# CSMaus/DefectDetection_viaObjectDetection

Hardware: AMD Instinct MI355X
Metric: images/sec @640x640 b32 YOLOv8s-seg (higher is better)
Workload: dtype fp16; 1 GPU; YOLOv8s-seg inference (forward + NMS + masks), 32 synthetic 640x640 B-scans per GPU per step, nc=1, seeded synthetic weights; pipelined throughput, 2 batch(es) in flight (ms_per_step is the step period, not a latency); inputs rotate over 8 HBM-resident batches (300 MiB); input_batches=8, per_gpu_batch=32, global_batch=32, parallelism=batch-sharded x1, no collective, max_det=300, engines_in_flight=2, stream_lanes_per_engine=1

## Files before the change

defectdetection_viaobjectdetection_amd/_capi.py:

```python
from __future__ import annotations

import ctypes as C
import os

_HERE = os.path.dirname(os.path.abspath(__file__))
LIB_PATH = os.path.join(_HERE, "lib", "libmi355yolo.so")


class M355Error(RuntimeError):
    """Raised when a libmi355yolo call returns a negative status."""


class ModelDesc(C.Structure):
    _fields_ = [("scale", C.c_int), ("nc", C.c_int), ("in_h", C.c_int), ("in_w", C.c_int),
                ("max_batch", C.c_int)]


class ConvInfo(C.Structure):
    _fields_ = [("name", C.c_char * 64), ("cin", C.c_int), ("cout", C.c_int), ("k", C.c_int),
                ("stride", C.c_int), ("has_bn", C.c_int), ("transposed", C.c_int), ("act", C.c_int),
                ("groups", C.c_int)]


class OpInfo(C.Structure):
# ... 95 lines not shown
    "m355_get_raw_head": (C.c_int, [_P, C.POINTER(_P), C.POINTER(C.c_int)]),
    "m355_copy_raw_head": (C.c_int, [_P, C.c_int, _P, _P]),
    "m355_set_keep_raw": (C.c_int, [_P, C.c_int]),
    "m355_postprocess": (C.c_int, [_P, _P, _P, C.c_int, C.c_float, C.c_float, C.c_int, _P, _P, _P, _P]),
    "m355_conv2d_fwd": (C.c_int, [_P, C.c_int, C.c_int, C.c_int, C.c_int, _P, _P, C.c_int, C.c_int, C.c_int,
                                  C.c_int, _P, _P, C.c_int, C.c_int, _P]),
    "m355_c2f_c32_fwd": (C.c_int, [_P, C.c_int, C.c_int, C.c_int, _P, _P, _P, _P, _P, _P, C.c_int, _P, _P]),
    "m355_bneck_pair_fwd": (C.c_int, [_P, C.c_int, C.c_int, C.c_int, C.c_int, C.c_int, _P, _P, _P, _P, C.c_int, _P, C.c_int, _P]),
    "m355_conv3x3_blockdiag_fwd": (C.c_int, [_P, C.c_int, C.c_int, C.c_int, C.c_int, C.c_int, _P, _P, _P, _P, _P, C.c_int, C.c_int, _P]),
    "m355_planes_diag_pack": (C.c_long, [C.c_int, _P, _P, _P, _P, C.c_long]),
    "m355_s2c64_cv1_fwd": (C.c_int, [_P, C.c_int, C.c_int, C.c_int, _P, _P, _P, _P, _P, _P]),
    "m355_stem_s2c32_cv1_fwd": (C.c_int, [_P, C.c_int, C.c_int, C.c_int, _P, _P, _P, _P, _P, _P, _P, C.c_int, _P]),
    "m355_proto_phase_fwd": (C.c_int, [_P, C.c_int, C.c_int, C.c_int, _P, _P, _P, _P, _P, _P, _P, _P]),
    "m355_head_tail_fwd": (C.c_int, [_P, C.c_int, C.c_int, C.c_int, C.c_int, C.c_float, _P, _P, _P, _P, _P, _P, _P, C.c_int, C.c_int, _P]),
    "m355_tal_assign_launch": (C.c_int, [_P, _P, _P, _P, _P, _P, C.c_int32, C.c_int32, C.c_int32, C.c_int32, _P, _P, _P, _P, _P, _P]),
    "m355_conv2d_dgrad": (C.c_int, [_P, C.c_int, C.c_int, C.c_int, C.c_int, _P, C.c_int, C.c_int, C.c_int, _P, _P]),
    "m355_conv2d_wgrad": (C.c_int, [_P, _P, C.c_int, C.c_int, C.c_int, C.c_int, C.c_int, C.c_int, C.c_int, _P, _P]),
    "m355_bn_silu_train_fwd": (C.c_int, [_P, C.c_int, C.c_int, C.c_int, C.c_int, _P, _P, C.c_float, C.c_int, _P, _P, _P, _P, _P]),
    "m355_bn_silu_train_bwd": (C.c_int, [_P, _P, C.c_int, C.c_int, C.c_int, C.c_int, _P, _P, _P, _P, C.c_int, _P, _P, _P, _P]),
    "m355_bn_workspace_floats": (C.c_size_t, [C.c_int]),
    "m355_wgrad_workspace_bytes": (C.c_size_t, [C.c_int32, C.c_int32, C.c_int32, C.c_int32, C.c_int32, C.c_int32]),
    "m355_grad_sumsq_workspace_floats": (C.c_size_t, []),
    "m355_convt2x2_fwd": (C.c_int, [_P, C.c_int, C.c_int, C.c_int, C.c_int, _P, _P, C.c_int, _P, _P]),
    "m355_stem_fwd": (C.c_int, [_P, C.c_int, C.c_int, C.c_int, _P, _P, C.c_int, _P, _P]),
    "m355_stem6_fwd": (C.c_int, [_P, C.c_int, C.c_int, C.c_int, _P, _P, C.c_int, _P, _P]),
    "m355_dwconv3x3_fwd": (C.c_int, [_P, C.c_int, C.c_int, C.c_int, C.c_int, C.c_int, _P, _P, C.c_int, _P, C.c_int, _P]),
    "m355_psa_attn_fwd": (C.c_int, [_P, C.c_int, C.c_int, C.c_int, C.c_int, C.c_int, C.c_int, _P, _P, _P, _P]),
    "m355_sppf_pool": (C.c_int, [_P, C.c_int, C.c_int, C.c_int, C.c_int, _P, _P]),
    "m355_upsample2x": (C.c_int, [_P, C.c_int, C.c_int, C.c_int, C.c_int, _P, _P]),
    "m355_head_decode": (C.c_int, [_P, C.c_int, C.c_int, C.c_int, C.c_int, _P, _P]),
    "m355_head_decode_ex": (C.c_int, [_P, C.c_int, C.c_int, C.c_int, C.c_int, C.c_int, _P, _P]),
    "m355_nms": (C.c_int, [_P, C.c_int, C.c_int, C.c_int, C.c_int, C.c_float, C.c_float, C.c_int, _P, _P, _P]),
    "m355_conv_launch": (C.c_int, [C.POINTER(ConvLaunchArgs), _P]),
    "m355_wgrad_launch": (C.c_int, [C.POINTER(WgradLaunchArgs), _P]),
    "m355_bn_train_fwd_launch": (C.c_int, [_P, C.c_int64, C.c_int32, C.c_int32, _P, _P, C.c_float, C.c_int32, _P, C.c_int32,
                                           _P, C.c_int32, _P, _P, _P, _P, _P, C.c_float, _P]),
    "m355_bn_train_bwd_launch": (C.c_int, [_P, _P, C.c_int64, C.c_int32, C.c_int32, C.c_int32, _P, _P, _P, _P, C.c_int32,
                                           _P, C.c_int32, _P, _P, _P]),
    "m355_adamw_step": (C.c_int, [_P, _P, _P, _P, _P, _P, C.c_int64, C.c_float, C.c_float, C.c_float, C.c_float, C.c_float,
                                  C.c_float, C.c_int32, C.c_float, C.c_float, _P]),
    "m355_sgd_step": (C.c_int, [_P, _P, _P, _P, _P, C.c_int64, C.c_float, C.c_float, C.c_float, C.c_int32, C.c_float,
                                C.c_float, C.c_float, _P]),
    "m355_grad_sumsq": (C.c_int, [_P, C.c_int64, _P, _P]),
    "m355_augment": (C.c_int, [_P, _P, _P, C.c_int32, C.c_int32, C.c_int32, _P]),
    "m355_augment_ex_workspace_bytes": (C.c_size_t, [C.c_int32, C.c_int32, C.c_int32]),
    "m355_augment_ex": (C.c_int, [_P, C.c_int32, C.POINTER(AugExParams), C.POINTER(AugPoly), C.c_int32, _F, C.c_int32, _P, C.c_int64,
                                  _P, C.c_int32, C.c_int32, C.c_int32, _P]),
    "m355_msda_forward": (C.c_int, [_P, C.c_int32, C.c_int32, C.c_int32, C.c_int32, _P, C.c_int32, _P, _P, _P, C.c_int32,
                                    C.c_int32, C.c_int32, _P, _P]),
    "m355_msda_module_forward": (C.c_int, [_P, C.c_int32, C.c_int32, C.c_int32, C.c_int32, _P, C.c_int32, _P, _P, _P, _P,
                                           C.c_int32, C.c_int32, C.c_float, _P, _P]),
    "m355_dfine_decode": (C.c_int, [_P, _P, _P, _P, C.c_int64, C.c_int32, C.c_float, C.c_int32, _P]),
    "m355_msda_backward_workspace_bytes": (C.c_size_t, [C.c_int32, C.c_int32, C.c_int32, C.c_int32]),
    "m355_msda_backward": (C.c_int, [_P, _P, C.c_int32, C.c_int32, C.c_int32, C.c_int32, _P, C.c_int32, _P, _P, _P, C.c_int32,
                                     C.c_int32, C.c_int32, _P, _P, _P, _P, C.c_int64, _P]),
    "m355_msda_module_backward": (C.c_int, [_P, _P, C.c_int32, C.c_int32, C.c_int32, C.c_int32, _P, C.c_int32, _P, _P, _P, _P,
                                            C.c_int32, C.c_int32, C.c_float, _P, _P, _P, _P, _P, C.c_int64, _P]),
    "m355_dfine_decode_backward": (C.c_int, [_P, _P, _P, _P, _P, _P, C.c_int64, C.c_int32, C.c_float, C.c_int32, _P]),
    "m355_dfine_match_workspace_bytes": (C.c_size_t, [C.c_int32, C.c_int32, C.c_int32]),
    "m355_dfine_match": (C.c_int, [_P, _P, C.c_int32, C.c_int32, C.c_int32, _P, _P, _P, _P, C.c_float, C.c_float, C.c_float,
                                   C.c_float, C.c_float, C.c_int32, _P, C.c_int64, _P, _P, _P, C.c_int32, _P, _P]),
    "m355_dfine_postprocess": (C.c_int, [_P, _P, C.c_int32, C.c_int32, C.c_int32, _P, C.c_float, _P, _P, _P, _P, _P]),
    "m355_dfine_preprocess": (C.c_int, [_P, C.c_int64, _P, _P, C.c_int32, _P, _P, C.c_int32, _P, _P, C.c_int64, _P, C.c_int32, C.c_int32,
                                        _P, C.c_int64, _P, _P]),
    "m355_dfine_select_workspace_bytes": (C.c_size_t, [C.c_int32, C.c_int32]),
    "m355_dfine_select_forward": (C.c_int, [_P, _P, _P, C.c_int32, C.c_int32, C.c_int32, C.c_int32, C.c_int32, _P, C.c_int64, _P, _P, _P,
# ... 119 lines not shown
```

defectdetection_viaobjectdetection_amd/csrc/common.h:

```cpp
#pragma once
#include <hip/hip_runtime.h>
#include <stdint.h>

namespace m355 {

typedef _Float16 half_t;
typedef _Float16 half8 __attribute__((ext_vector_type(8)));
typedef _Float16 half4 __attribute__((ext_vector_type(4)));
typedef _Float16 half2v __attribute__((ext_vector_type(2)));
typedef float float4v __attribute__((ext_vector_type(4)));

constexpr int BK = 64;

struct ConvArgs {
  const half_t* x;
  long x_bstride;
  int ldx;
  int Hi, Wi, Cin;
  const half_t* w;
  int Kpad;
  const float* bias;
  void* y;
  long y_bstride;
  int ldy;
// ... 2 lines not shown
  const half_t* res;
  long r_bstride;
  int ldr;
  int ksize, stride, pad;
  int M;
  int act;
  int out_f32;
  int convt_co;
  const half_t* zero;
  int tmode;
  int dbg;
  unsigned long long* stamps;
  const half_t* x2;
  long x2_bstride;
  int ldx2;
  int csplit;
  int phase;
  const half_t* w2;
  const float* bias2;
  int cout2;
  float* dec_preds;
  int dec_A, dec_level_off, dec_nc, dec_nm, dec_keep_raw;
  float dec_stride;
  int w_rows;
  int* tileq;
  const half_t* wf;
  const half_t* wf2;
  int bias_lds;
};

constexpr int DBG_ABLATE_IGEMM = 1 | 2 | 8 | 32, DBG_ABLATE_HALO = 1 | 2 | 4 | 8, DBG_ABLATE_M32 = 1 | 2 | 4;
inline bool conv_probe_wanted(const ConvArgs& a, int ablation_bits) { return a.stamps || (a.dbg & ablation_bits); }

enum { TILE_AUTO = -1, TILE_128x128 = 0, TILE_64x128 = 1, TILE_32x256 = 2, TILE_64x256 = 3, TILE_64x128W8 = 5, TILE_HALO = 16, TILE_HALO8W = 17, TILE_HALO4W = 18, TILE_HALOWIDE = 19, TILE_C32 = 20, TILE_SLAB = 25, TILE_M32 = 26, TILE_M32_128 = 27, TILE_M32_64x16 = 28, TILE_M32_64x8 = 29, TILE_W1 = 32, TILE_PLANES = 33 };


int launch_conv_igemm(const ConvArgs& a, int force_tile, hipStream_t s);
int conv_pick_tile(int cout, long M);
int conv_cout_pad(int cout);
int conv_kpad(int cin, int ksize);
inline bool conv_rows_covered(const ConvArgs& a, int bch) {
  const int need = (a.Cout + bch - 1) / bch * bch;
  return need <= (a.w_rows > 0 ? a.w_rows : conv_cout_pad(a.Cout));
}
bool conv_forced_tile_extent(int tile, int cout, int* bch, int* bpx);

bool conv3x3_halo_ok(const ConvArgs& a);
int launch_conv3x3_halo(const ConvArgs& a, int variant, hipStream_t s);
int conv3x3_halo_pick(const ConvArgs& a, bool no_wide, bool no_m32);
bool conv3x3_wide_ok(const ConvArgs& a);
int launch_conv3x3_wide(const ConvArgs& a, hipStream_t s);
bool conv3x3_m32_ok(const ConvArgs& a);
int launch_conv3x3_m32(const ConvArgs& a, int which, hipStream_t s);
bool conv_s2c32_cv1_ok(const ConvArgs& a);
int launch_conv_s2c32_cv1(const ConvArgs& a, hipStream_t s);
bool conv3x3_slab_ok(const ConvArgs& a);
int launch_conv3x3_slab(const ConvArgs& a, hipStream_t s);
struct MsdaLevels { int L; int lh[8], lw[8], lstart[8], pend[8]; };
int launch_msda(const float* value, const float* loc, const float* attn, float* out, int B, int S, int H, int Q, int P,
                const MsdaLevels& lv, int discrete, hipStream_t s, const float* ref = nullptr, float offset_scale = 0.f);
int launch_dfine_decode(const float* dist, const float* project, const float* ref, float* boxes, long n, int nbins1,
                        float reg_scale, int clamp01, hipStream_t s, bool guard = false);
int dfine_tfuse_max_t();
int dfine_noobject_max_q();
int launch_dfine_tfuse_forward(const float* fused, const float* scores, const float* ctx, int T, int Q, int D, float* out, float* stats,
                               hipStream_t s);
int launch_dfine_tfuse_backward(const float* g, const float* fused, const float* scores, const float* stats, int T, int Q, int D,
                                float* d_fused, float* d_scores, hipStream_t s);
int launch_dfine_guard_logits(const float* cls, const float* an, long rows, int C1, float bound, float* out, hipStream_t s);
int launch_dfine_guard_logits_backward(const float* g, const float* cls, const float* an, long rows, int C1, float bound, float* d_cls,
                                       float* d_an, hipStream_t s);
int launch_dfine_noobject_forward(const float* x, int T, int Q, int C, int cls, float* out, hipStream_t s);
int launch_dfine_noobject_backward(const float* g, const float* x, int T, int Q, int C, int cls, float* dx, hipStream_t s);
size_t dfine_consistency_workspace_bytes(int T, long N);
int launch_dfine_consistency_forward(const float* a, int T, long N, float* work, float* out, hipStream_t s);
int launch_dfine_consistency_backward(const float* g, const float* a, int T, long N, float* da, hipStream_t s);
size_t dfine_match_workspace_bytes(int B, int Q, int nmax);
int launch_dfine_match(const float* logits, const float* boxes, int B, int Q, int C, const long long* labels, const float* tboxes,
                       const int* d_offsets, int T, int nmax, float class_cost, float bbox_cost, float giou_cost, float alpha,
                       float gamma, int focal, void* work, float* cost_out, long long* rows, long long* cols, int kmax, int* flags,
                       hipStream_t s);
int launch_dfine_postprocess(const float* logits, const float* boxes, int B, int Q, int C, const float* sizes, float threshold,
// ... 281 lines not shown
```

defectdetection_viaobjectdetection_amd/csrc/engine.hip:

```cpp
#include <math.h>
#include <stdio.h>
#include <stdlib.h>
#include <string.h>

#include <algorithm>
#include <string>
#include <vector>

#include "../../include/mi355yolo.h"
#include "common.h"
#include "engine_types.h"
#include "switches.h"
#include "weight_pack.h"

using namespace m355;

thread_local std::string m355::g_err;

namespace {

void fuse_conv_cv1(m355_engine* e) {
  if (e->sw.no_cvfuse) return;
  for (size_t i = 0; i < e->ops.size(); ++i) {
    Op& oi = e->ops[i];
// ... 296 lines not shown
}

HeadTailArgs head_tail_args(const m355_engine* e, const Op& op, int B, float* preds) {
  const PhysConv& p = e->phys[op.conv];
  const Tensor& ti = e->tensors[op.in.t];
  HeadTailArgs a{};
  a.x = ti.p; a.ldx = ti.C; a.M = (long)B * ti.H * ti.W; a.HW = ti.H * ti.W; a.W = ti.W;
  a.stride = (float)(e->desc.in_h / ti.H);
  a.A = e->A; a.level_off = op.level_off; a.nc = e->nc; a.nm = e->nm;
  a.wf = p.wf; a.bias = p.bias; a.preds = preds;
  return a;
}

bool head_tail_layout(const m355_engine* e, const PhysConv& p) {
  return p.diag && p.logical.size() == 3 && p.cin == 224 && p.cout == 64 + e->nc + e->nm && e->nm == 32 && e->nc <= 32 &&
         e->convs[p.logical[0]].cin == 64 && e->convs[p.logical[1]].cin == 128;
}

void plan_route(m355_engine* e, Op& op, const ConvArgs& a) {
  const PlanSwitches& sw = e->sw;
  PhysConv& p = e->phys[op.conv];
  const Tensor& ti = e->tensors[op.in.t];
  if (op.kind == OP_PHASE) {
    op.tile = p.cout % 128 == 0 ? TILE_128x128 : TILE_64x128;
    if (p.l3 >= 0 && p.cin == 128 && p.cout == 128 && p.cout2 == 32 && ti.H % 8 == 0 && ti.W % 16 == 0 && !sw.no_protor)
      op.route = R_PROTOR;
    return;
  }
  const bool conv = op.kind == OP_CONV;
  op.tile = conv_pick_tile(a.Cout, a.M);
  if (a.ksize == 1 && op.tile == TILE_128x128 && sw.k1_tile >= 0) op.tile = sw.k1_tile;
  if (op.decode) op.tile = TILE_128x128;
  if (conv && conv3x3_halo_ok(a) && !sw.no_halo) op.route = R_HALO;
  const bool m32 = op.route == R_HALO && conv3x3_halo_pick(a, proc_switches().no_wide, proc_switches().no_m32) == TILE_M32;
  if (conv && conv3x3_c32_ok(a) && !sw.no_c32) op.route = R_C32;
  if (conv && op.out_ext == 0 && p.l3 < 0 && !p.diag && op.res.t < 0 && !op.decode && (op.in2.t < 0 || !sw.no_w1_split) &&
      conv1x1_wreg_ok(a) && !sw.no_w1)
    op.route = R_W1;
  if (conv && op.route != R_HALO && op.route != R_C32 && conv3x3_slab_ok(a) && !sw.no_slab) op.route = R_SLAB;
  const bool planes_s2 = p.k == 3 && p.stride == 2 && op.res.t < 0 && op.in2.t < 0 && !sw.no_planes_s2;
  const bool planes_m64 = m32 && a.Cout <= 64 && op.res.t < 0 && op.in2.t < 0 && !sw.no_planes_m64;
  if (conv && (op.route == R_SLAB || planes_s2 || planes_m64) && op.out_ext == 0 && p.l3 < 0 && !p.diag && !sw.no_planes) {
    PlanesArgs pa = planes_args(e, op, e->desc.max_batch, 0);
    pa.wfb = (const half_t*)1;
    if (conv3x3_planes_ok(pa)) {
      op.route = R_PLANES;
      p.planes = 1;
    }
  }
  if (conv && op.out_ext == 1 && !op.decode && head_tail_layout(e, p) && ti.C == 224 && op.in.off == 0 && op.raw_off == 0 &&
      a.Ho * a.Wo >= 32 && !sw.no_headtail) {
    op.headtail = 1;
    ++e->headtail_n;
  }
  if (conv && p.l3 >= 0 && p.k == 3 && p.stride == 2 && p.cin == 32 && p.cout == 64 && p.cout2 == 64 && a.Ho % 8 == 0 &&
      a.Wo % 16 == 0 && !sw.no_s2c32)
    op.route = R_S2C32;
  if (conv && p.l3 >= 0 && p.k == 3 && p.stride == 2 && p.cin == 64 && p.cout == 128 && p.cout2 == 128 && a.Ho % 8 == 0 &&
      a.Wo % 8 == 0 && !sw.no_s2c64)
    op.route = R_S2C64;
}

void conv_label(const m355_engine* e, Op& op, const ConvArgs& a) {
  static const char* tile_names[] = {"128x128", "64x128", "32x256", "64x256"};
  const PhysConv& p = e->phys[op.conv];
  char* k = op.kernel;
  const size_t n = sizeof(op.kernel);
  const char* ch = a.Cout > 64 ? "128ch" : "64ch";
  switch (op.route) {
    case R_IGEMM:
      if (op.kind == OP_PHASE) snprintf(k, n, "conv_igemm<%s,k2,phase%s>", tile_names[op.tile], p.l3 >= 0 ? "+1x1" : "");
      else snprintf(k, n, "conv_igemm<%s,k%d%s>", tile_names[op.tile], a.ksize, p.l3 >= 0 ? "+1x1" : op.decode ? "+decode" : "");
      break;
    case R_HALO: {
      const int pick = conv3x3_halo_pick(a, proc_switches().no_wide, proc_switches().no_m32);
      if (pick == TILE_HALOWIDE) snprintf(k, n, "conv3x3_wide<128ch,16x16px>");
      else if (pick == TILE_M32) snprintf(k, n, "conv3x3_m32<%s,8x16px>", ch);
      else snprintf(k, n, "conv3x3_halo<%s>", ch);
      break;
    }
    case R_C32: snprintf(k, n, "conv3x3_c32<32ch,16x16px>"); break;
    case R_SLAB: snprintf(k, n, "conv3x3_slab<64ch,rows>"); break;
    case R_W1: snprintf(k, n, "conv1x1_wreg<K%d,%dch>", p.cin, a.Cout % 256 == 0 ? 256 : 128); break;
    case R_PLANES: snprintf(k, n, p.stride == 2 ? "conv3x3_planes<64ch,rows,s2>" : "conv3x3_planes<64ch,rows>"); break;
    case R_S2C32: snprintf(k, n, "conv3x3_s2c32<8x16px>+1x1"); break;
    case R_S2C64: snprintf(k, n, "conv3x3_s2c64<8x8px>+1x1"); break;
    case R_PROTOR: snprintf(k, n, "proto_phase_wreg<8x16px>"); break;
  }
}

void annotate_ops(m355_engine* e) {
  for (Op& op : e->ops) {
    if (op.conv >= 0) snprintf(op.layer, sizeof(op.layer), "%s", e->convs[e->phys[op.conv].logical[0]].name);
    if (op.kind == OP_CONV || op.kind == OP_CONVT || op.kind == OP_PHASE) {
      const ConvArgs a = conv_args(e, op, e->desc.max_batch, 0, nullptr, nullptr);
      plan_route(e, op, a);
      conv_label(e, op, a);
    }
    switch (op.kind) {
      case OP_STEM: {
        const PhysConv& p = e->phys[op.conv];
        const Tensor& to = e->tensors[op.out.t];
        snprintf(op.kernel, sizeof(op.kernel), "stem_conv<k3s2,u8,mfma>");
        op.flops = 2.0 * to.H * to.W * p.cout * 27;
        op.bytes = (double)op.Hi * op.Wi * 3 + (double)to.H * to.W * p.cout * 2;
        op.wbytes = 28.0 * p.cout * 4;
        if (p.k == 6) {
          snprintf(op.kernel, sizeof(op.kernel), "stem6_s2<k6s2p2,u8,mfma>");
          op.flops = 2.0 * to.H * to.W * p.cout * 108;
          op.wbytes = (double)p.cout * (128 * 2 + 4);
        }
        break;
      }
// ... 434 lines not shown
        rc = launch_stem(stem_args(e, op, Bq, b0, d_in), s);
        break;
      }
      case OP_CONV:
      case OP_CONVT:
      case OP_PHASE: {
        if (op.headtail && e->headtail_active && !b0) {
          rc = launch_head_tail(head_tail_args(e, op, Bq, d_preds), s);
          break;
        }
        if (op.diag_on) {
          rc = launch_conv3x3_blockdiag(diag_args(e, oi, Bq, b0), s);
          break;
        }
        ConvArgs a = conv_args(e, op, Bq, b0, d_preds, d_protos);
        if (op.kind != OP_PHASE) a.tileq = proc_switches().static_tiles ? nullptr : e->tileq + 4 * oi;
        if (op.stemfuse >= 0) {
          const StemArgs sa = stem_args(e, e->ops[op.stemfuse], Bq, b0, d_in);
          const bool stem2 = !live_no_stem2();
          if (stem2 && stem_s2c32_v2_ok(a, sa)) {
            rc = launch_stem_s2c32_v2(a, sa, s);
            break;
          }
          if (stem_s2c32_ok(a, sa)) {
            rc = launch_stem_s2c32(a, sa, s);
            break;
          }
          rc = launch_stem(sa, s);
          if (rc != 0) break;
        }
        switch (op.route) {
          case R_IGEMM: rc = launch_conv_igemm(a, op.tile, s); break;
          case R_HALO: rc = launch_conv3x3_halo(a, 0, s); break;
          case R_C32: rc = launch_conv3x3_c32(a, s); break;
          case R_SLAB: rc = launch_conv3x3_slab(a, s); break;
          case R_W1: rc = conv1x1_wreg_ok(a) ? launch_conv1x1_wreg(a, s) : launch_conv_igemm(a, TILE_AUTO, s); break;
          case R_PLANES: {
            const PlanesArgs pa = planes_args(e, op, Bq, b0);
            rc = (pa.wfb && conv3x3_planes_ok(pa)) ? launch_conv3x3_planes(pa, s)
                 : a.stride == 2 ? launch_conv_igemm(a, TILE_AUTO, s)
                 : conv3x3_slab_ok(a) ? launch_conv3x3_slab(a, s) : launch_conv3x3_halo(a, 0, s);
            break;
          }
          case R_S2C32: rc = conv_s2c32_cv1_ok(a) ? launch_conv_s2c32_cv1(a, s) : launch_conv_igemm(a, op.tile, s); break;
          case R_S2C64: rc = conv_s2c64_cv1_ok(a) ? launch_conv_s2c64_cv1(a, s) : launch_conv_igemm(a, op.tile, s); break;
          case R_PROTOR: rc = proto_phase_wreg_ok(a) ? launch_proto_phase_wreg(a, s) : launch_conv_igemm(a, op.tile, s); break;
        }
        break;
      }
      case OP_C2F32: {
        const Tensor& ti = e->tensors[op.in.t];
        const Tensor& to = e->tensors[op.out.t];
        const PhysConv &pa = e->phys[op.conv], &pb = e->phys[op.conv2], &pc = e->phys[op.conv3];
        C2fC32Args a{};
        a.x_bstride = (long)ti.H * ti.W * ti.C; a.ldx = ti.C; a.H = ti.H; a.W = ti.W; a.B = Bq;
        a.x = ti.p + op.in.off + b0 * a.x_bstride;
        a.wa = pa.w; a.wb = pb.w; a.wc = pc.w; a.waf = pa.wf; a.wbf = pb.wf2; a.kpad_a = pa.Kpad; a.kpad_b = pb.Kpad; a.kpad_c = pc.Kpad;
        a.ba = pa.bias; a.bb = pb.bias; a.bc = pc.bias;
        a.y_bstride = (long)to.H * to.W * to.C; a.ldy = to.C;
        a.y = to.p + op.out.off + b0 * a.y_bstride;
        a.shortcut = op.shortcut;
        rc = launch_c2f_c32(a, s);
        break;
      }
      case OP_PAIR: {
        const PlanesArgs a = planes_args(e, op, Bq, b0);
// ... 218 lines not shown
```

defectdetection_viaobjectdetection_amd/csrc/engine_types.h:

```cpp
#pragma once
#include <string>
#include <vector>

#include "../../include/mi355yolo.h"
#include "common.h"
#include "switches.h"
#include "weight_pack.h"

#pragma GCC visibility push(hidden)

namespace m355 {

struct Tensor {
  int H = 0, W = 0, C = 0;
  half_t* p = nullptr;
};

struct Slice {
  int t = -1, off = 0, c = 0;
};

enum OpKind { OP_STEM, OP_CONV, OP_CONVT, OP_PHASE, OP_POOL, OP_UP, OP_DECODE, OP_ADOWN, OP_C2F32, OP_PAIR, OP_DWCONV, OP_PSA_ATTN };

enum Route {
  R_IGEMM,
  R_HALO,
  R_C32,
  R_SLAB,
  R_W1,
  R_PLANES,
  R_S2C32,
  R_S2C64,
  R_PROTOR,
};

struct Op {
  OpKind kind;
  int conv = -1;
  int conv2 = -1, conv3 = -1;
  int shortcut = 0;
  int heads = 0;
  Slice in, out, res;
  Slice in2;
  Slice out2;
  int out_ext = 0;
  int raw_off = 0;
  int level_off = 0;
  int Hi = 0, Wi = 0;
  char kernel[48] = {0};
  char layer[64] = {0};
  double flops = 0;
  double bytes = 0;
  double wbytes = 0;
  Route route = R_IGEMM;
  int tile = -1;
  int decode = 0;
  int headtail = 0;
  int diag_n = 0;
  int diag_on = 0;
  int stemfuse = -1;
  bool fused_away = false;
  int lane = 0;
  std::vector<int> wait_ops;
  bool record = false;
};

// ... 86 lines not shown
```

defectdetection_viaobjectdetection_amd/csrc/op_entries.hip:

```cpp
#include <math.h>
#include <stdio.h>
#include <stdlib.h>
#include <string.h>

#include <string>
#include <vector>

#include "../../include/mi355yolo.h"
#include "common.h"
#include "launch_util.h"
#include "switches.h"
#include "weight_pack.h"

using namespace m355;

namespace {

struct DevBuf {
  std::vector<void*> p;
  ~DevBuf() { for (void* q : p) (void)hipFree(q); }
  void* alloc(size_t bytes) {
    void* d = nullptr;
    if (hipMalloc(&d, bytes + 16) != hipSuccess) return nullptr;
    p.push_back(d);
// ... 651 lines not shown
  if (d_class_mask && nc > 1024) return set_err(M355_ERR_INVALID, "a class set covers at most 1024 classes");
  return nms_entry(d_preds, B, A, nc, nm, conf, iou, max_det, agnostic, d_class_mask, d_dets, d_counts, stream);
}

int m355_proto_masks_native(const float* d_dets, const int* d_counts, const void* d_protos, int B, int max_det, int mh,
                            int mw, const int32_t* h_orig_hw, const float* d_boxes, const int64_t* h_offsets,
                            uint8_t* d_out, void* stream) {
  if (!d_dets || !d_counts || !d_protos || !d_boxes || !h_orig_hw || !h_offsets)
    return set_err(M355_ERR_INVALID, "null pointer");
  const int rc = launch_proto_masks_native(d_dets, d_counts, (const half_t*)d_protos, B, max_det, mh, mw, h_orig_hw,
                                           d_boxes, h_offsets, d_out, (hipStream_t)stream);
  if (rc == -1)
    return set_err(M355_ERR_INVALID, "proto_masks_native: bad argument (shape, max_det, offset table, alignment or null output)");
  return rc == 0 ? M355_OK : set_err(M355_ERR_HIP, "native mask launch failed: " + std::to_string(rc));
}

int m355_letterbox_u8(const uint8_t* d_src, const m355_letterbox_image* h_table, int n, int net_h, int net_w,
                      uint8_t* d_out, void* stream) {
  if (!d_src || !h_table || !d_out) return set_err(M355_ERR_INVALID, "letterbox: null pointer");
  const int rc = launch_letterbox_u8(d_src, h_table, n, net_h, net_w, d_out, (hipStream_t)stream);
  if (rc == -1)
    return set_err(M355_ERR_INVALID, "letterbox: bad argument (n, net shape, output alignment, image or window size, offset table)");
  return rc == 0 ? M355_OK : set_err(M355_ERR_HIP, "letterbox launch failed: " + std::to_string(rc));
}

int m355_proto_masks(const float* d_dets, const int* d_counts, const void* d_protos, int B, int max_det, int mh,
                     int mw, int in_h, int in_w, uint8_t* d_masks, void* stream) {
  if (!d_dets || !d_counts || !d_protos || !d_masks) return set_err(M355_ERR_INVALID, "null pointer");
  const int rc = launch_proto_masks(d_dets, d_counts, (const half_t*)d_protos, B, max_det, 32, mh, mw, in_h, in_w,
                                    d_masks, (hipStream_t)stream);
  return rc == 0 ? M355_OK : set_err(M355_ERR_HIP, "mask launch failed: " + std::to_string(rc));
}

int m355_conv_launch(const m355_conv_args* c, void* stream) {
  if (!c || !c->x || !c->w_packed || !c->bias || !c->y || !c->zero_page) return set_err(M355_ERR_INVALID, "null pointer");
  ConvArgs a{};
  a.x = (const half_t*)c->x; a.x_bstride = c->x_bstride; a.ldx = c->ldx; a.Hi = c->hi; a.Wi = c->wi; a.Cin = c->cin;
  a.w = (const half_t*)c->w_packed; a.Kpad = c->kpad; a.bias = c->bias;
  a.y = c->y; a.y_bstride = c->y_bstride; a.ldy = c->ldy; a.Ho = c->ho; a.Wo = c->wo; a.Cout = c->cout;
  a.res = (const half_t*)c->res; a.r_bstride = c->r_bstride; a.ldr = c->ldr;
  a.ksize = c->ksize; a.stride = c->stride; a.pad = c->pad; a.M = c->batch * c->ho * c->wo;
  a.act = c->act; a.out_f32 = c->out_f32; a.convt_co = c->convt_co; a.tmode = c->tmode;
  a.zero = (const half_t*)c->zero_page;
  if (c->convt_co > 0 && c->tmode == 0 && c->ksize == 1 && c->res)
    return set_err(M355_ERR_INVALID, "ConvTranspose (convt_co > 0, ksize 1) takes no residual");
  if (c->tmode == 2) {
    a.tmode = 0;
    a.phase = dgrad_phase_form(c->convt_co, c->cin, c->res != nullptr);
    if (!a.phase)
      return set_err(M355_ERR_INVALID, "tmode 2 needs convt_co % 64 == 0, or 128 % convt_co == 0 with convt_co >= 16 and no res "
                                       "(use the tmode 1 gather)");
  }
  int rc;
  const bool train_w1 = !proc_switches().no_train_w1;
  const bool train_c32 = !proc_switches().no_train_c32;
  if (a.phase == 2 && dgrad_s2c32_ok(a))
    rc = launch_dgrad_s2c32(a, (hipStream_t)stream);
  else if (!a.tmode && conv3x3_halo_ok(a))
    rc = launch_conv3x3_halo(a, 0, (hipStream_t)stream);
  else if (train_w1 && !a.tmode && conv1x1_wreg_ok(a))
    rc = launch_conv1x1_wreg(a, (hipStream_t)stream);
  else if (train_c32 && !a.tmode && conv3x3_c32_ok(a) && conv_rows_covered(a, 32))
    rc = launch_conv3x3_c32(a, (hipStream_t)stream);
  else
    rc = launch_conv_igemm(a, TILE_AUTO, (hipStream_t)stream);
  return rc == 0 ? M355_OK : set_err(M355_ERR_HIP, "conv launch failed: " + std::to_string(rc));
}

int m355_wgrad_launch(const m355_wgrad_args* w, void* stream) {
  if (!w || !w->dz || !w->x || !w->dw || !w->zero_page) return set_err(M355_ERR_INVALID, "null pointer");
  const int rc = launch_conv_wgrad((const half_t*)w->dz, w->dz_bstride, w->lddz, (const half_t*)w->x, w->x_bstride, w->ldx,
                                   w->batch, w->hi, w->wi, w->cin, w->ho, w->wo, w->cout, w->ksize, w->stride, w->pad,
                                   w->dw, (const half_t*)w->zero_page, w->ws, (size_t)(w->ws_bytes < 0 ? 0 : w->ws_bytes),
                                   (hipStream_t)stream);
  if (rc == -3) return set_err(M355_ERR_INVALID, "wgrad workspace missing or smaller than m355_wgrad_workspace_bytes()");
  return rc == 0 ? M355_OK : set_err(M355_ERR_HIP, "wgrad launch failed: " + std::to_string(rc));
// ... 180 lines not shown
```

defectdetection_viaobjectdetection_amd/csrc/switches.h:

```cpp
#pragma once

namespace m355 {

struct ProcSwitches {
  bool no_fast_epi, no_wide, no_m32, no_bias_lds, static_tiles, no_persist, stem_gather;
  int persist, halo_variant, smallm;
  bool c2f_noprio;
  const char* c2f_stamps;
  int c32_waste, c32_slots, m32_slots, wide_slots, wide_stagger;
  int s2c32_dbg, s2c32_ring, s2c64_prio, protor_prio;
  const char *s2c32_stamps, *s2c64_stamps, *protor_stamps;
  int stem2_nxb;
  bool no_stemfuse;
  int sppf_minblocks, mask_dbg, mask_tile;
  bool no_dgrad_s2c32, no_wgrad_stem, no_wgrad_s2c32, no_wgrad3, no_train_w1, no_train_c32;
  int wgrad_blocks, w2_blocks_x2, wgrad3_shrink, wgrad3_blocks, wgrad3_mintiles;
  long wgrad3_slabmb;
};
const ProcSwitches& proc_switches();

struct PlanSwitches {
  bool no_c2f32, no_pair, no_protofuse, no_protofuse3, no_upfuse;
  bool no_headdiag, headdiag_l0;
  int lane_plan[4];
  bool no_cvfuse, decfuse, no_lanes, no_subbatch;
  bool no_stemfuse;
  int subbatch, subbatch_ops;
  bool no_protor, no_halo, no_c32, no_w1_split, no_w1, no_slab, no_planes_s2, no_planes_m64, no_planes, no_headtail, no_s2c32,
      no_s2c64;
  int k1_tile;
  long headtail_maxm;
};
PlanSwitches read_plan_switches();

bool live_no_stem2();
bool live_no_dgrad_phases();
bool live_pair64();
const char* live_stamps_path();
int live_bneck_reps();

}
```

defectdetection_viaobjectdetection_amd/csrc/switches.hip:

```cpp
#include "switches.h"

#include <limits.h>
#include <stdlib.h>

namespace m355 {

namespace {

bool env_set(const char* name) { return getenv(name) != nullptr; }
long env_int(const char* name, long unset) {
  const char* v = getenv(name);
  return v ? atol(v) : unset;
}

ProcSwitches read_proc_switches() {
  ProcSwitches v{};
  v.no_fast_epi = env_set("M355_NO_FAST_EPI");
  v.no_wide = env_set("M355_NO_WIDE");
  v.no_m32 = env_set("M355_NO_M32");
  v.no_bias_lds = env_set("M355_NO_BIAS_LDS");
  v.static_tiles = env_set("M355_STATIC_TILES");
  v.no_persist = env_set("M355_NO_PERSIST");
  v.stem_gather = env_set("M355_STEM_GATHER");
  v.persist = env_int("M355_PERSIST", 0);
// ... 34 lines not shown
}

}

const ProcSwitches& proc_switches() {
  static const ProcSwitches v = read_proc_switches();
  return v;
}

PlanSwitches read_plan_switches() {
  PlanSwitches v{};
  v.no_c2f32 = env_set("M355_NO_C2F32");
  v.no_pair = env_set("M355_NO_PAIR");
  v.no_protofuse = env_set("M355_NO_PROTOFUSE");
  v.no_protofuse3 = env_set("M355_NO_PROTOFUSE3");
  v.no_upfuse = env_set("M355_NO_UPFUSE");
  v.no_headdiag = env_set("M355_NO_HEADDIAG");
  v.headdiag_l0 = env_set("M355_HEADDIAG_L0");
  const int lanes[4] = {1, 2, 2, 0};
  const char* lp = getenv("M355_LANE_PLAN");
  for (int i = 0; i < 4; ++i) {
    if (lp && (lp[i] < '0' || lp[i] > '3')) lp = nullptr;
    v.lane_plan[i] = lp ? lp[i] - '0' : lanes[i];
  }
  v.no_cvfuse = env_set("M355_NO_CVFUSE");
  v.decfuse = env_set("M355_DECFUSE");
  v.no_lanes = env_set("M355_NO_LANES");
  v.no_subbatch = env_set("M355_NO_SUBBATCH");
  v.no_stemfuse = env_set("M355_NO_STEMFUSE");
  v.subbatch = env_int("M355_SUBBATCH", 0);
  v.subbatch_ops = env_int("M355_SUBBATCH_OPS", INT_MAX);
  v.no_protor = env_set("M355_NO_PROTOR");
  v.no_halo = env_set("M355_NO_HALO");
  v.no_c32 = env_set("M355_NO_C32");
  v.no_w1_split = env_set("M355_NO_W1_SPLIT");
  v.no_w1 = env_set("M355_NO_W1");
  v.no_slab = env_set("M355_NO_SLAB");
  v.no_planes_s2 = env_set("M355_NO_PLANES_S2");
  v.no_planes_m64 = env_set("M355_NO_PLANES_M64");
  v.no_planes = env_set("M355_NO_PLANES");
  v.no_headtail = env_set("M355_NO_HEADTAIL");
  v.no_s2c32 = env_set("M355_NO_S2C32");
  v.no_s2c64 = env_set("M355_NO_S2C64");
  v.k1_tile = env_int("M355_K1_TILE", -1);
  v.headtail_maxm = env_int("M355_HEADTAIL_MAXM", 0);
  return v;
}

bool live_no_stem2() { return env_set("M355_NO_STEM2"); }
bool live_no_dgrad_phases() { return env_set("M355_NO_DGRAD_PHASES"); }
bool live_pair64() { return env_set("M355_PAIR64"); }
const char* live_stamps_path() { return getenv("M355_STAMPS"); }
int live_bneck_reps() { return env_int("M355_BNECK_REPS", 0); }

}
```

include/mi355yolo.h:

```cpp
#ifndef MI355YOLO_H_
#define MI355YOLO_H_

#include <stddef.h>
#include <stdint.h>

#ifdef __cplusplus
extern "C" {
#endif

typedef struct m355_engine m355_engine;

typedef enum {
  M355_OK = 0,
  M355_ERR_INVALID = -1,
  M355_ERR_NO_DEVICE = -2,
  M355_ERR_HIP = -3,
  M355_ERR_STATE = -4,
  M355_ERR_NOMEM = -5
} m355_status;

typedef struct {
  int scale;
  int nc;
  int in_h, in_w;
// ... 98 lines not shown
int m355_sppf_pool(const void* d_x, int B, int H, int W, int C, void* d_y, void* stream);
int m355_upsample2x(const void* d_x, int B, int H, int W, int C, void* d_y, void* stream);
int m355_head_decode(const float* d_raw, int B, int in_h, int in_w, int nc, float* d_preds, void* stream);
int m355_head_decode_ex(const float* d_raw, int B, int in_h, int in_w, int nc, int nm, float* d_preds, void* stream);
int m355_nms(const float* d_preds, int B, int A, int nc, int nm, float conf, float iou, int max_det,
             float* d_dets, int* d_counts, void* stream);
int m355_nms_ex(const float* d_preds, int B, int A, int nc, int nm, float conf, float iou, int max_det, int agnostic,
                const uint32_t* d_class_mask, float* d_dets, int* d_counts, void* stream);
int m355_proto_masks_native(const float* d_dets, const int* d_counts, const void* d_protos, int B, int max_det, int mh,
                            int mw, const int32_t* h_orig_hw, const float* d_boxes, const int64_t* h_offsets,
                            uint8_t* d_out, void* stream);
typedef struct {
  int64_t offset;
  int32_t h, w;
  int32_t uh, uw;
  int32_t top, left;
} m355_letterbox_image;
int m355_letterbox_u8(const uint8_t* d_src, const m355_letterbox_image* h_table, int n, int net_h, int net_w,
                      uint8_t* d_out, void* stream);
int m355_proto_masks(const float* d_dets, const int* d_counts, const void* d_protos, int B, int max_det,
                     int mh, int mw, int in_h, int in_w, uint8_t* d_masks, void* stream);

typedef struct {
  const void* x; int64_t x_bstride; int32_t ldx; int32_t hi, wi, cin;
  const void* w_packed; int32_t kpad;
  const float* bias;
  void* y; int64_t y_bstride; int32_t ldy; int32_t ho, wo, cout;
  const void* res; int64_t r_bstride; int32_t ldr;
  int32_t ksize, stride, pad, batch;
  int32_t act, out_f32, convt_co, tmode;
  const void* zero_page;
} m355_conv_args;
int m355_conv_launch(const m355_conv_args* a, void* stream);

typedef struct {
  const void* dz; int64_t dz_bstride; int32_t lddz;
  const void* x; int64_t x_bstride; int32_t ldx;
  int32_t hi, wi, cin, ho, wo, cout;
  int32_t ksize, stride, pad, batch;
  float* dw;
  const void* zero_page;
  float* ws; int64_t ws_bytes;
} m355_wgrad_args;
size_t m355_wgrad_workspace_bytes(int32_t batch, int32_t ho, int32_t wo, int32_t cin, int32_t cout, int32_t ksize);
int m355_wgrad_launch(const m355_wgrad_args* a, void* stream);

int m355_bn_train_fwd_launch(const void* z, int64_t npix, int32_t ldz, int32_t C, const float* gamma, const float* beta,
                             float eps, int32_t act, void* y, int32_t ldy, const void* res, int32_t ldr, float* mean,
                             float* invstd, float* ws, float* running_mean, float* running_var, float momentum,
                             void* stream);
int m355_bn_train_bwd_launch(const void* z, const void* dy, int64_t npix, int32_t ldz, int32_t lddy, int32_t C,
                             const float* mean, const float* invstd, const float* gamma, const float* beta, int32_t act,
                             void* dz, int32_t lddz, float* dbeta_dgamma, float* ws, void* stream);
int m355_sppf_pool_launch(const void* x, int64_t x_bstride, int32_t ldx, void* y, int64_t y_bstride, int32_t ldy,
                          int32_t B, int32_t H, int32_t W, int32_t C, void* stream);
int m355_sppf_pool_form(int32_t B, int32_t H, int32_t W, int32_t C, int32_t ldy);
typedef struct m355_repack_job {
  const void* src;
  void* dst;
  int32_t n[4];
  int64_t ss[4];
  int64_t ds[4];
  int32_t block0;
  int32_t pad_;
} m355_repack_job;
int m355_repack_launch(const m355_repack_job* d_jobs, const int32_t* d_block_job, int32_t nblocks, void* stream);
// ... 272 lines not shown
```

Baseline: 19350 images/s.

## Add persistent 64-channel 3x3 conv kernel with LDS-resident weights and double-buffered patches

Adds a persistent 3x3 convolution kernel for 64-in/64-out channel layers. It keeps all nine weight taps in LDS for the whole launch and double-buffers 18x18 input patches via async DMA while MFMA runs on the current tile. The router sends eligible halo-route convs with at least 25600 output pixels to it. The aim is to stop reloading weights per tile and to hide input latency, at the cost of one block per CU (large LDS footprint) and a grid sized to the CU count. An explicit tile-launch API entry point is also added.

New measurement: 19370 images/s (median of 2 runs). Within noise of the previous version (+0.1%).

```diff
diff --git a/defectdetection_viaobjectdetection_amd/_capi.py b/defectdetection_viaobjectdetection_amd/_capi.py
--- a/defectdetection_viaobjectdetection_amd/_capi.py
+++ b/defectdetection_viaobjectdetection_amd/_capi.py
@@ -151,6 +151,7 @@
     "m355_head_decode_ex": (C.c_int, [_P, C.c_int, C.c_int, C.c_int, C.c_int, C.c_int, _P, _P]),
     "m355_nms": (C.c_int, [_P, C.c_int, C.c_int, C.c_int, C.c_int, C.c_float, C.c_float, C.c_int, _P, _P, _P]),
     "m355_conv_launch": (C.c_int, [C.POINTER(ConvLaunchArgs), _P]),
+    "m355_conv_launch_tile": (C.c_int, [C.POINTER(ConvLaunchArgs), C.c_int, C.c_int, _P]),
     "m355_wgrad_launch": (C.c_int, [C.POINTER(WgradLaunchArgs), _P]),
     "m355_bn_train_fwd_launch": (C.c_int, [_P, C.c_int64, C.c_int32, C.c_int32, _P, _P, C.c_float, C.c_int32, _P, C.c_int32,
                                            _P, C.c_int32, _P, _P, _P, _P, _P, C.c_float, _P]),
diff --git a/defectdetection_viaobjectdetection_amd/csrc/common.h b/defectdetection_viaobjectdetection_amd/csrc/common.h
--- a/defectdetection_viaobjectdetection_amd/csrc/common.h
+++ b/defectdetection_viaobjectdetection_amd/csrc/common.h
@@ -58,7 +58,7 @@
 constexpr int DBG_ABLATE_IGEMM = 1 | 2 | 8 | 32, DBG_ABLATE_HALO = 1 | 2 | 4 | 8, DBG_ABLATE_M32 = 1 | 2 | 4;
 inline bool conv_probe_wanted(const ConvArgs& a, int ablation_bits) { return a.stamps || (a.dbg & ablation_bits); }
 
-enum { TILE_AUTO = -1, TILE_128x128 = 0, TILE_64x128 = 1, TILE_32x256 = 2, TILE_64x256 = 3, TILE_64x128W8 = 5, TILE_HALO = 16, TILE_HALO8W = 17, TILE_HALO4W = 18, TILE_HALOWIDE = 19, TILE_C32 = 20, TILE_SLAB = 25, TILE_M32 = 26, TILE_M32_128 = 27, TILE_M32_64x16 = 28, TILE_M32_64x8 = 29, TILE_W1 = 32, TILE_PLANES = 33 };
+enum { TILE_AUTO = -1, TILE_128x128 = 0, TILE_64x128 = 1, TILE_32x256 = 2, TILE_64x256 = 3, TILE_64x128W8 = 5, TILE_HALO = 16, TILE_HALO8W = 17, TILE_HALO4W = 18, TILE_HALOWIDE = 19, TILE_C32 = 20, TILE_SLAB = 25, TILE_M32 = 26, TILE_M32_128 = 27, TILE_M32_64x16 = 28, TILE_M32_64x8 = 29, TILE_W1 = 32, TILE_PLANES = 33, TILE_RES64 = 34 };
 
 
 int launch_conv_igemm(const ConvArgs& a, int force_tile, hipStream_t s);
@@ -74,6 +74,11 @@
 bool conv3x3_halo_ok(const ConvArgs& a);
 int launch_conv3x3_halo(const ConvArgs& a, int variant, hipStream_t s);
 int conv3x3_halo_pick(const ConvArgs& a, bool no_wide, bool no_m32);
+constexpr long CONV3X3_RES64_MIN_PIXELS = 25600;
+bool conv3x3_res64_takes(const ConvArgs& a);
+bool conv3x3_res64_ok(const ConvArgs& a);
+int conv3x3_res64_prepare();
+int launch_conv3x3_res64(const ConvArgs& a, hipStream_t s, int max_blocks = 0);
 bool conv3x3_wide_ok(const ConvArgs& a);
 int launch_conv3x3_wide(const ConvArgs& a, hipStream_t s);
 bool conv3x3_m32_ok(const ConvArgs& a);
diff --git a/defectdetection_viaobjectdetection_amd/csrc/conv3x3_res64.hip b/defectdetection_viaobjectdetection_amd/csrc/conv3x3_res64.hip
--- /dev/null
+++ b/defectdetection_viaobjectdetection_amd/csrc/conv3x3_res64.hip
@@ -0,0 +1,227 @@
+#include "common.h"
+#include "device_prims.h"
+#include "launch_util.h"
+
+namespace m355 {
+namespace {
+
+constexpr int TS = 16, TH = 16;
+constexpr int PW = TS + 2, PH = TH + 2;
+constexpr int ROWB = 128;
+constexpr int NWAVES = 8;
+constexpr int MT = 4, NT = 2;
+constexpr int PGROUPS = (PH * PW + 7) / 8;
+constexpr int PATCH_BYTES = PGROUPS * 8 * ROWB;
+constexpr int P_IT = (PGROUPS + NWAVES - 1) / NWAVES;
+constexpr int WTAP = 64 * ROWB;
+constexpr int LDS_BYTES = 2 * PATCH_BYTES + 9 * WTAP;
+static_assert(LDS_BYTES <= 160 * 1024, "one CU's LDS");
+static_assert((PATCH_BYTES & 64) == 0, "the K-slice bit of an address is the same in both patch buffers");
+
+__global__ __launch_bounds__(NWAVES * 64, 1) void conv3x3_res64_kernel(const ConvArgs a, int tiles_x, int tiles_y, int ntiles) {
+  extern __shared__ __attribute__((aligned(16))) char smem[];
+  char* const wbase = smem + 2 * PATCH_BYTES;
+
+  const int tid = threadIdx.x;
+  const int lane = tid & 63;
+  const int wave = __builtin_amdgcn_readfirstlane(tid >> 6);
+  const int lrow = lane >> 3;
+  const int cc = (lane & 7) ^ lrow;
+  const int H = a.Hi, W = a.Wi;
+  const bool late = wave >= 4;
+
+  {
+    const int R = wave * 8 + lrow;
+    const int mt = R >> 4, r = R & 15;
+    const int chl = (mt >> 1) * 32 + (r >> 2) * 8 + (mt & 1) * 4 + (r & 3);
+    const half_t* wr = a.w + (long)chl * a.Kpad + cc * 8;
+#pragma unroll
+    for (int t = 0; t < 9; ++t) glds16(wr + t * 64, wbase + t * WTAP + wave * 1024);
+  }
+
+  auto decode = [&](int vb, int& tb, int& ty0, int& tx0) __attribute__((always_inline)) {
+    const int xcd = vb & 7, q = ntiles >> 3, r = ntiles & 7;
+    int rest = (xcd < r ? xcd * (q + 1) : r * (q + 1) + (xcd - r) * q) + (vb >> 3);
+    const int tx = rest % tiles_x;
+    rest /= tiles_x;
+    const int ty = rest % tiles_y;
+    tb = rest / tiles_y;
+    ty0 = ty * TH;
+    tx0 = tx * TS;
+  };
+  const __amdgpu_buffer_rsrc_t rs_x = __builtin_amdgcn_make_buffer_rsrc(
+      (void*)a.x, 0, (int)(((long)(ntiles / (tiles_x * tiles_y)) - 1) * a.x_bstride + (long)H * W * a.ldx) * 2, 0x00020000);
+  const int img_stride = (int)a.x_bstride * 2;
+  auto issue_patch = [&](int tb, int ty0, int tx0, int buf) __attribute__((always_inline)) {
+    const int soff = tb * img_stride;
+#pragma unroll
+    for (int i = 0; i < P_IT; ++i) {
+      const int j = wave + NWAVES * i;
+      if (i < P_IT - 1 || j < PGROUPS) {
+        const int p = 8 * j + lrow;
+        const int py = p / PW, px = p - py * PW;
+        const int iy = ty0 - 1 + py, ix = tx0 - 1 + px;
+        const bool ok = p < PH * PW && (unsigned)iy < (unsigned)H && (unsigned)ix < (unsigned)W;
+        dma16(rs_x, ok ? ((iy * W + ix) * a.ldx + cc * 8) * 2 : (int)0x80000000, soff, smem + buf * PATCH_BYTES + j * 1024);
+      }
+    }
+  };
+
+  const int l15 = lane & 15, g = lane >> 4;
+  const int aoff = l15 * ROWB + ((g ^ (l15 & 7)) << 4);
+  int boff[9][NT];
+#pragma unroll
+  for (int t = 0; t < 9; ++t)
+#pragma unroll
+    for (int nt = 0; nt < NT; ++nt) {
+      const int p = (wave * NT + nt + t / 3) * PW + l15 + t % 3;
+      boff[t][nt] = (p << 7) + ((g ^ (p & 7)) << 4);
+    }
+
+  float4v bv[MT / 2][2];
+  {
+    const float* bp = a.bias + g * 8;
+#pragma unroll
+    for (int sg = 0; sg < MT / 2; ++sg) {
+      bv[sg][0] = *(const float4v*)(bp + sg * 32);
+      bv[sg][1] = *(const float4v*)(bp + sg * 32 + 4);
+    }
+  }
+
+  float4v acc[MT][NT];
+  auto epilogue = [&](int eb, int ey0, int ex0) __attribute__((always_inline)) {
+    const long pix0 = (long)(ey0 + wave * NT) * W + ex0 + l15;
+    const int cho = g * 8;
+    half_t* yp = (half_t*)a.y + (long)eb * a.y_bstride + pix0 * a.ldy + cho;
+    const long ystep = (long)W * a.ldy;
+    if (a.res) {
+      const half_t* rp = a.res + (long)eb * a.r_bstride + pix0 * a.ldr + cho;
+      const long rstep = (long)W * a.ldr;
+      if (a.act) conv_epilogue_fast<MT, NT, true, true>(acc, bv, yp, ystep, rp, rstep);
+      else conv_epilogue_fast<MT, NT, false, true>(acc, bv, yp, ystep, rp, rstep);
+    } else {
+      if (a.act) conv_epilogue_fast<MT, NT, true, false>(acc, bv, yp, ystep, nullptr, 0);
+      else conv_epilogue_fast<MT, NT, false, false>(acc, bv, yp, ystep, nullptr, 0);
+    }
+  };
+
+  int vb = blockIdx.x;
+  int cb, cy0, cx0;
+  decode(vb, cb, cy0, cx0);
+  issue_patch(cb, cy0, cx0, 0);
+  if (vb + (int)gridDim.x < ntiles) {
+    int nb, ny0, nx0;
+    decode(vb + gridDim.x, nb, ny0, nx0);
+    issue_patch(nb, ny0, nx0, 1);
+  }
+  asm volatile("s_waitcnt vmcnt(0) lgkmcnt(0)" ::: "memory");
+  __builtin_amdgcn_s_waitcnt(WAITCNT_VM_LGKM0(0));
+  __builtin_amdgcn_s_barrier();
+
+  auto tile_barrier = [&]() __attribute__((always_inline)) {
+    vb += gridDim.x;
+    if (vb < ntiles) __builtin_amdgcn_s_barrier();
+  };
+  int buf = 0;
+  auto advance = [&]() __attribute__((always_inline)) {
+    if (vb < ntiles) {
+      decode(vb, cb, cy0, cx0);
+      if (vb + (int)gridDim.x < ntiles) {
+        int nb, ny0, nx0;
+        decode(vb + gridDim.x, nb, ny0, nx0);
+        issue_patch(nb, ny0, nx0, buf);
+      }
+      buf ^= 1;
+    }
+  };
+
+#define M355_SB __builtin_amdgcn_sched_barrier(0);
+#define M355_MF(AF, BF, mt, nt) acc[mt][nt] = __builtin_amdgcn_mfma_f32_16x16x32_f16(AF[mt], BF[nt], acc[mt][nt], 0, 0, 0);
+#define M355_HALF(AF, BF, m0) M355_MF(AF, BF, m0, 0) M355_MF(AF, BF, m0, 1) M355_MF(AF, BF, m0 + 1, 0) M355_MF(AF, BF, m0 + 1, 1)
+  while (vb < ntiles) {
+    const char* const pb = smem + buf * PATCH_BYTES;
+    const int eb = cb, ey0 = cy0, ex0 = cx0;
+#pragma unroll
+    for (int mt = 0; mt < MT; ++mt)
+#pragma unroll
+      for (int nt = 0; nt < NT; ++nt) acc[mt][nt] = float4v{0.f, 0.f, 0.f, 0.f};
+    half8 af0[MT], bf0[NT], af1[MT], bf1[NT];
+#pragma unroll
+    for (int mt = 0; mt < MT; ++mt) af0[mt] = *(const half8*)(wbase + aoff + mt * 2048);
+#pragma unroll
+    for (int nt = 0; nt < NT; ++nt) bf0[nt] = *(const half8*)(pb + boff[0][nt]);
+#pragma unroll
+    for (int t = 0; t < 9; ++t) {
+      const char* const wt = wbase + t * WTAP;
+      M355_SB
+#pragma unroll
+      for (int mt = 0; mt < MT; ++mt) af1[mt] = *(const half8*)(wt + (aoff ^ 64) + mt * 2048);
+#pragma unroll
+      for (int nt = 0; nt < NT; ++nt) bf1[nt] = *(const half8*)(pb + (boff[t][nt] ^ 64));
+      M355_SB
+      M355_HALF(af0, bf0, 0)
+      M355_HALF(af0, bf0, 2)
+      M355_SB
+      if (t < 8) {
+#pragma unroll
+        for (int mt = 0; mt < MT; ++mt) af0[mt] = *(const half8*)(wt + WTAP + aoff + mt * 2048);
+#pragma unroll
+        for (int nt = 0; nt < NT; ++nt) bf0[nt] = *(const half8*)(pb + boff[t + 1][nt]);
+      }
+      M355_SB
+      M355_HALF(af1, bf1, 0)
+      M355_HALF(af1, bf1, 2)
+    }
+    M355_SB
+    asm volatile("s_waitcnt vmcnt(0) lgkmcnt(0)" ::: "memory");
+    if (late) tile_barrier();
+    epilogue(eb, ey0, ex0);
+    if (!late) tile_barrier();
+    advance();
+  }
+#undef M355_SB
+#undef M355_MF
+#undef M355_HALF
+}
+
+int g_res64_ready = 0;
+int g_res64_err = 0;
+int g_res64_grid = 0;
+
+}
+
+int conv3x3_res64_prepare() {
+  if (g_res64_ready) return g_res64_ready > 0 ? 0 : g_res64_err;
+  int e = prepare_kernel((const void*)conv3x3_res64_kernel, LDS_BYTES);
+  const int cus = num_cus();
+  if (!e && cus < 8) e = -2;
+  g_res64_grid = cus & ~7;
+  g_res64_err = e;
+  g_res64_ready = e ? -1 : 1;
+  return e;
+}
+
+bool conv3x3_res64_takes(const ConvArgs& a) {
+  if (a.Cin != 64 || a.Cout != 64 || !conv3x3_halo_ok(a)) return false;
+  if (a.Hi % TH || a.Wi % TS || a.M < a.Hi * a.Wi || !conv_rows_covered(a, 64)) return false;
+  if (a.res && a.ldr % 8) return false;
+  const long B = a.M / (a.Hi * a.Wi);
+  return ((B - 1) * a.x_bstride + (long)a.Hi * a.Wi * a.ldx) * 2 < (1L << 31);
+}
+
+bool conv3x3_res64_ok(const ConvArgs& a) { return conv3x3_res64_takes(a) && (long)a.M >= CONV3X3_RES64_MIN_PIXELS; }
+
+int launch_conv3x3_res64(const ConvArgs& a, hipStream_t s, int max_blocks) {
+  if (!conv3x3_res64_takes(a)) return -1;
+  if (const int e = conv3x3_res64_prepare()) return e;
+  const int tiles_x = a.Wi / TS, tiles_y = a.Hi / TH;
+  const int B = a.M / (a.Ho * a.Wo);
+  const int ntiles = B * tiles_y * tiles_x;
+  int slots = g_res64_grid;
+  if (max_blocks > 0 && max_blocks < slots) slots = max_blocks < 8 ? 8 : (max_blocks & ~7);
+  const int grid = ntiles <= slots ? ntiles : slots;
+  hipLaunchKernelGGL(conv3x3_res64_kernel, dim3(grid), dim3(NWAVES * 64), LDS_BYTES, s, a, tiles_x, tiles_y, ntiles);
+  return (int)hipGetLastError();
+}
+
+}
diff --git a/defectdetection_viaobjectdetection_amd/csrc/engine.hip b/defectdetection_viaobjectdetection_amd/csrc/engine.hip
--- a/defectdetection_viaobjectdetection_amd/csrc/engine.hip
+++ b/defectdetection_viaobjectdetection_amd/csrc/engine.hip
@@ -352,12 +352,13 @@
   if (a.ksize == 1 && op.tile == TILE_128x128 && sw.k1_tile >= 0) op.tile = sw.k1_tile;
   if (op.decode) op.tile = TILE_128x128;
   if (conv && conv3x3_halo_ok(a) && !sw.no_halo) op.route = R_HALO;
+  if (op.route == R_HALO && !sw.no_res64 && conv3x3_res64_ok(a) && conv3x3_res64_prepare() == 0) op.route = R_RES64;
   const bool m32 = op.route == R_HALO && conv3x3_halo_pick(a, proc_switches().no_wide, proc_switches().no_m32) == TILE_M32;
   if (conv && conv3x3_c32_ok(a) && !sw.no_c32) op.route = R_C32;
   if (conv && op.out_ext == 0 && p.l3 < 0 && !p.diag && op.res.t < 0 && !op.decode && (op.in2.t < 0 || !sw.no_w1_split) &&
       conv1x1_wreg_ok(a) && !sw.no_w1)
     op.route = R_W1;
-  if (conv && op.route != R_HALO && op.route != R_C32 && conv3x3_slab_ok(a) && !sw.no_slab) op.route = R_SLAB;
+  if (conv && op.route != R_HALO && op.route != R_RES64 && op.route != R_C32 && conv3x3_slab_ok(a) && !sw.no_slab) op.route = R_SLAB;
   const bool planes_s2 = p.k == 3 && p.stride == 2 && op.res.t < 0 && op.in2.t < 0 && !sw.no_planes_s2;
   const bool planes_m64 = m32 && a.Cout <= 64 && op.res.t < 0 && op.in2.t < 0 && !sw.no_planes_m64;
   if (conv && (op.route == R_SLAB || planes_s2 || planes_m64) && op.out_ext == 0 && p.l3 < 0 && !p.diag && !sw.no_planes) {
@@ -399,6 +400,7 @@
       else snprintf(k, n, "conv3x3_halo<%s>", ch);
       break;
     }
+    case R_RES64: snprintf(k, n, "conv3x3_res64<64ch>"); break;
     case R_C32: snprintf(k, n, "conv3x3_c32<32ch,16x16px>"); break;
     case R_SLAB: snprintf(k, n, "conv3x3_slab<64ch,rows>"); break;
     case R_W1: snprintf(k, n, "conv1x1_wreg<K%d,%dch>", p.cin, a.Cout % 256 == 0 ? 256 : 128); break;
@@ -899,6 +901,7 @@
         switch (op.route) {
           case R_IGEMM: rc = launch_conv_igemm(a, op.tile, s); break;
           case R_HALO: rc = launch_conv3x3_halo(a, 0, s); break;
+          case R_RES64: rc = conv3x3_res64_takes(a) ? launch_conv3x3_res64(a, s) : launch_conv3x3_halo(a, 0, s); break;
           case R_C32: rc = launch_conv3x3_c32(a, s); break;
           case R_SLAB: rc = launch_conv3x3_slab(a, s); break;
           case R_W1: rc = conv1x1_wreg_ok(a) ? launch_conv1x1_wreg(a, s) : launch_conv_igemm(a, TILE_AUTO, s); break;
diff --git a/defectdetection_viaobjectdetection_amd/csrc/engine_types.h b/defectdetection_viaobjectdetection_amd/csrc/engine_types.h
--- a/defectdetection_viaobjectdetection_amd/csrc/engine_types.h
+++ b/defectdetection_viaobjectdetection_amd/csrc/engine_types.h
@@ -32,6 +32,7 @@
   R_S2C32,
   R_S2C64,
   R_PROTOR,
+  R_RES64,
 };
 
 struct Op {
diff --git a/defectdetection_viaobjectdetection_amd/csrc/op_entries.hip b/defectdetection_viaobjectdetection_amd/csrc/op_entries.hip
--- a/defectdetection_viaobjectdetection_amd/csrc/op_entries.hip
+++ b/defectdetection_viaobjectdetection_amd/csrc/op_entries.hip
@@ -707,8 +707,7 @@
   return rc == 0 ? M355_OK : set_err(M355_ERR_HIP, "mask launch failed: " + std::to_string(rc));
 }
 
-int m355_conv_launch(const m355_conv_args* c, void* stream) {
-  if (!c || !c->x || !c->w_packed || !c->bias || !c->y || !c->zero_page) return set_err(M355_ERR_INVALID, "null pointer");
+static ConvArgs conv_launch_args(const m355_conv_args* c) {
   ConvArgs a{};
   a.x = (const half_t*)c->x; a.x_bstride = c->x_bstride; a.ldx = c->ldx; a.Hi = c->hi; a.Wi = c->wi; a.Cin = c->cin;
   a.w = (const half_t*)c->w_packed; a.Kpad = c->kpad; a.bias = c->bias;
@@ -717,6 +716,24 @@
   a.ksize = c->ksize; a.stride = c->stride; a.pad = c->pad; a.M = c->batch * c->ho * c->wo;
   a.act = c->act; a.out_f32 = c->out_f32; a.convt_co = c->convt_co; a.tmode = c->tmode;
   a.zero = (const half_t*)c->zero_page;
+  return a;
+}
+
+int m355_conv_launch_tile(const m355_conv_args* c, int tile, int max_blocks, void* stream) {
+  if (!c || !c->x || !c->w_packed || !c->bias || !c->y || !c->zero_page) return set_err(M355_ERR_INVALID, "null pointer");
+  if (c->tmode || c->convt_co || c->batch < 1 || c->ho < 1 || c->wo < 1) return set_err(M355_ERR_INVALID, "a plain forward convolution only");
+  if (tile != TILE_RES64 && (tile < TILE_HALO || tile > TILE_M32_64x8 || tile == TILE_C32))
+    return set_err(M355_ERR_INVALID, "unknown 3x3 tile id " + std::to_string(tile));
+  const ConvArgs a = conv_launch_args(c);
+  const int rc = tile == TILE_RES64 ? launch_conv3x3_res64(a, (hipStream_t)stream, max_blocks)
+                                    : launch_conv3x3_halo(a, tile - TILE_HALO, (hipStream_t)stream);
+  if (rc == -1) return set_err(M355_ERR_INVALID, "conv launch failed: -1");
+  return rc == 0 ? M355_OK : set_err(M355_ERR_HIP, "conv launch failed: " + std::to_string(rc));
+}
+
+int m355_conv_launch(const m355_conv_args* c, void* stream) {
+  if (!c || !c->x || !c->w_packed || !c->bias || !c->y || !c->zero_page) return set_err(M355_ERR_INVALID, "null pointer");
+  ConvArgs a = conv_launch_args(c);
   if (c->convt_co > 0 && c->tmode == 0 && c->ksize == 1 && c->res)
     return set_err(M355_ERR_INVALID, "ConvTranspose (convt_co > 0, ksize 1) takes no residual");
   if (c->tmode == 2) {
diff --git a/defectdetection_viaobjectdetection_amd/csrc/switches.h b/defectdetection_viaobjectdetection_amd/csrc/switches.h
--- a/defectdetection_viaobjectdetection_amd/csrc/switches.h
+++ b/defectdetection_viaobjectdetection_amd/csrc/switches.h
@@ -26,7 +26,7 @@
   bool no_cvfuse, decfuse, no_lanes, no_subbatch;
   bool no_stemfuse;
   int subbatch, subbatch_ops;
-  bool no_protor, no_halo, no_c32, no_w1_split, no_w1, no_slab, no_planes_s2, no_planes_m64, no_planes, no_headtail, no_s2c32,
+  bool no_protor, no_halo, no_res64, no_c32, no_w1_split, no_w1, no_slab, no_planes_s2, no_planes_m64, no_planes, no_headtail, no_s2c32,
       no_s2c64;
   int k1_tile;
   long headtail_maxm;
diff --git a/defectdetection_viaobjectdetection_amd/csrc/switches.hip b/defectdetection_viaobjectdetection_amd/csrc/switches.hip
--- a/defectdetection_viaobjectdetection_amd/csrc/switches.hip
+++ b/defectdetection_viaobjectdetection_amd/csrc/switches.hip
@@ -90,6 +90,7 @@
   v.subbatch_ops = env_int("M355_SUBBATCH_OPS", INT_MAX);
   v.no_protor = env_set("M355_NO_PROTOR");
   v.no_halo = env_set("M355_NO_HALO");
+  v.no_res64 = env_set("M355_NO_RES64");
   v.no_c32 = env_set("M355_NO_C32");
   v.no_w1_split = env_set("M355_NO_W1_SPLIT");
   v.no_w1 = env_set("M355_NO_W1");
diff --git a/include/mi355yolo.h b/include/mi355yolo.h
--- a/include/mi355yolo.h
+++ b/include/mi355yolo.h
@@ -154,6 +154,7 @@
   const void* zero_page;
 } m355_conv_args;
 int m355_conv_launch(const m355_conv_args* a, void* stream);
+int m355_conv_launch_tile(const m355_conv_args* a, int tile, int max_blocks, void* stream);
 
 typedef struct {
   const void* dz; int64_t dz_bstride; int32_t lddz;
```
